# zero-savvy/vimz

Measured on AMD Instinct MI355X. Metric: nova_folding_steps_per_sec, higher is better.
Workload: dtype u32 limbs (256-bit Montgomery integers over BN254 Fr/Fq)

## Files before the change

vimz_amd/csrc/ec_mem.hpp:

```cpp
#pragma once
#include <hip/hip_runtime.h>
#include "ec.hpp"

namespace vz {

template <class F>
__device__ __forceinline__ void load_words20(const uint32_t* __restrict__ p, F& a, F& b) {
  const uint4* q = reinterpret_cast<const uint4*>(p);
  const uint4 w0 = q[0], w1 = q[1], w2 = q[2], w3 = q[3], w4 = q[4];
  a.v[0] = w0.x; a.v[1] = w0.y; a.v[2] = w0.z; a.v[3] = w0.w; a.v[4] = w1.x; a.v[5] = w1.y; a.v[6] = w1.z; a.v[7] = w1.w; a.v[8] = w2.x;
  b.v[0] = w2.z; b.v[1] = w2.w; b.v[2] = w3.x; b.v[3] = w3.y; b.v[4] = w3.z; b.v[5] = w3.w; b.v[6] = w4.x; b.v[7] = w4.y; b.v[8] = w4.z;
}
template <class F>
__device__ __forceinline__ void store_words20(uint32_t* __restrict__ p, const F& a, const F& b) {
  uint4* q = reinterpret_cast<uint4*>(p);
  q[0] = make_uint4(a.v[0], a.v[1], a.v[2], a.v[3]); q[1] = make_uint4(a.v[4], a.v[5], a.v[6], a.v[7]);
  q[2] = make_uint4(a.v[8], 0u, b.v[0], b.v[1]); q[3] = make_uint4(b.v[2], b.v[3], b.v[4], b.v[5]);
  q[4] = make_uint4(b.v[6], b.v[7], b.v[8], 0u);
}
struct RawAffine { uint4 w0, w1, w2, w3; };
__device__ __forceinline__ RawAffine load_affine_raw(const uint32_t* __restrict__ bases, size_t idx) {
  const uint4* q = reinterpret_cast<const uint4*>(bases + (size_t)AFFINE_WORDS * idx);
  RawAffine r; r.w0 = q[0]; r.w1 = q[1]; r.w2 = q[2]; r.w3 = q[3]; return r;
}
template <class F>
__device__ __forceinline__ Affine<F> affine_of_raw(const RawAffine& a) {
  const uint32_t x[8] = {a.w0.x, a.w0.y, a.w0.z, a.w0.w, a.w1.x, a.w1.y, a.w1.z, a.w1.w}, y[8] = {a.w2.x, a.w2.y, a.w2.z, a.w2.w, a.w3.x, a.w3.y, a.w3.z, a.w3.w};
  Affine<F> r; r.x = F::pack(x); r.y = F::pack(y); return r;
}
template <class F>
__device__ __forceinline__ Affine<F> load_affine_at(const uint32_t* __restrict__ p) { return affine_of_raw<F>(load_affine_raw(p, 0)); }
template <class F>
__device__ __forceinline__ Affine<F> load_affine(const uint32_t* __restrict__ bases, size_t idx) { return load_affine_at<F>(bases + (size_t)AFFINE_WORDS * idx); }
template <class F>
__device__ __forceinline__ void store_affine_at(uint32_t* __restrict__ p, const Affine<F>& a) {
  uint32_t x[8], y[8]; a.x.unpack(x); a.y.unpack(y);
  uint4* q = reinterpret_cast<uint4*>(p);
  q[0] = make_uint4(x[0], x[1], x[2], x[3]); q[1] = make_uint4(x[4], x[5], x[6], x[7]);
  q[2] = make_uint4(y[0], y[1], y[2], y[3]); q[3] = make_uint4(y[4], y[5], y[6], y[7]);
}
template <class F>
__device__ __forceinline__ void store_affine(uint32_t* __restrict__ bases, size_t idx, const Affine<F>& a) { store_affine_at<F>(bases + (size_t)AFFINE_WORDS * idx, a); }
constexpr int XYZZ_HALF_WORDS = 2 * COORD_WORDS;
template <class F>
__device__ __forceinline__ void store_xyzz(uint32_t* __restrict__ base, size_t idx, const XYZZ<F>& p) {
  uint32_t* d = base + (size_t)XYZZ_WORDS * idx;
  store_words20(d, p.X, p.Y); store_words20(d + XYZZ_HALF_WORDS, p.ZZ, p.ZZZ);
}
template <class F>
__device__ __forceinline__ XYZZ<F> load_xyzz(const uint32_t* __restrict__ base, size_t idx) {
  const uint32_t* d = base + (size_t)XYZZ_WORDS * idx;
  XYZZ<F> p; load_words20(d, p.X, p.Y); load_words20(d + XYZZ_HALF_WORDS, p.ZZ, p.ZZZ); return p;
}

template <class F> struct QuadRes { F c0, c1; XYZZ<F> full; uint32_t mode; };
template <int K, class F>
__device__ __forceinline__ F quad_bcast(const F& v) {
  F r;
#pragma unroll
  for (int i = 0; i < 9; i++) r.v[i] = (uint32_t)__builtin_amdgcn_update_dpp(0, (int)v.v[i], K * 0x55, 0xf, 0xf, true);
  return r;
}
template <class F>
__device__ __noinline__ void quad_add_rare(const XYZZ<F>* A, const XYZZ<F>* B, XYZZ<F>* out) { XYZZ<F> a = *A; add_full(a, *B); *out = a; }
template <class F>
__device__ __forceinline__ QuadRes<F> quad_add_compute(const XYZZ<F>* __restrict__ sh, uint32_t ia, uint32_t ib, bool active) {
  const int q = (int)(threadIdx.x & 3u);
  QuadRes<F> out; out.mode = 0;
  const XYZZ<F>& A = sh[ia]; const XYZZ<F>& B = sh[ib];
  const bool a_id = A.ZZ.is_zero(), b_id = B.ZZ.is_zero();
  auto sel = [](bool c, const F& x, const F& y) { F r; for (int i = 0; i < 9; i++) r.v[i] = c ? x.v[i] : y.v[i]; return r; };
  const F* px = q == 0 ? &A.X : q == 1 ? &B.X : q == 2 ? &A.Y : &B.Y;
  const F* py = q == 0 ? &B.ZZ : q == 1 ? &A.ZZ : q == 2 ? &B.ZZZ : &A.ZZZ;
  const F m1 = F::mul(*px, *py);
  F o1;
#pragma unroll
  for (int i = 0; i < 9; i++) o1.v[i] = (uint32_t)__builtin_amdgcn_update_dpp(0, (int)m1.v[i], 0xB1, 0xf, 0xf, true);
  const F lo = sel(q & 1, o1, m1), hi = sel(q & 1, m1, o1);
  const F PR = F::template sub<2>(hi, lo);
  const int pz = __builtin_amdgcn_update_dpp(0, (q == 0 && PR.is_zero_mod()) ? 1 : 0, 0x00, 0xf, 0xf, true);
  const F* pa = q == 1 ? &A.ZZ : &A.ZZZ; const F* pb = q == 1 ? &B.ZZ : &B.ZZZ;
  const F za = *pa, zb = *pb;
  const F m2 = F::mul(sel(q & 1, za, PR), sel(q & 1, zb, PR));
  const F PP = quad_bcast<0>(m2);
  const F Z12 = quad_bcast<1>(m2);
  const F m3 = F::mul(sel(q == 0, PR, sel(q == 1, lo, Z12)), PP);
  const F PPP = quad_bcast<0>(m3);
  const F Qv = quad_bcast<1>(m3);
  const F S1 = quad_bcast<2>(lo);
  const F X3 = F::template sub<4>(m2, F::add(PPP, F::dbl(Qv)));
  const F D = F::template sub<6>(Qv, X3);
  const F m4 = F::mul(sel(q == 0, S1, sel(q == 2, PR, m2)), sel(q == 2, D, PPP));
  const F Yb = quad_bcast<0>(m4);
  if (!active || b_id) return out;
  if (a_id) { out.mode = 1; out.c0 = q == 0 ? B.X : q == 1 ? B.Y : q == 2 ? B.ZZ : B.ZZZ; return out; }
  if (pz) {
    out.mode = 3;
    if (q == 0) { XYZZ<F> tmp; quad_add_rare<F>(&A, &B, &tmp); out.full = tmp; }
    return out;
  }
  out.mode = 2;
  if (q == 2) { out.c0 = X3; out.c1 = F::template sub<2>(m4, Yb); }
  if (q == 3) { out.c0 = m3; out.c1 = m4; }
  return out;
}
template <class F>
__device__ __forceinline__ void quad_add_store(XYZZ<F>* __restrict__ sh, uint32_t ia, const QuadRes<F>& r) {
  const int q = (int)(threadIdx.x & 3u);
  XYZZ<F>& A = sh[ia];
  if (r.mode == 1) { if (q == 0) A.X = r.c0; else if (q == 1) A.Y = r.c0; else if (q == 2) A.ZZ = r.c0; else A.ZZZ = r.c0; }
  else if (r.mode == 2) { if (q == 2) { A.X = r.c0; A.Y = r.c1; } else if (q == 3) { A.ZZ = r.c0; A.ZZZ = r.c1; } }
  else if (r.mode == 3 && q == 0) A = r.full;
}
template <class F, class Fd, class Fs>
__device__ __forceinline__ void quad_level(XYZZ<F>* __restrict__ sh, uint32_t count, Fd dst, Fs src) {
  const uint32_t e = threadIdx.x >> 2;
  const bool active = e < count;
  QuadRes<F> r; r.mode = 0;
  uint32_t ia = 0;
  const uint32_t wave0 = (uint32_t)__builtin_amdgcn_readfirstlane((int)(threadIdx.x & ~63u));
  if (wave0 < 4u * count) {
    ia = active ? dst(e) : 0u;
    const uint32_t ib = active ? src(e) : 0u;
    r = quad_add_compute<F>(sh, ia, ib, active);
  }
  __syncthreads();
  quad_add_store<F>(sh, ia, r);
  __syncthreads();
}

template <class F>
__device__ __forceinline__ void quad_tree256(XYZZ<F>* __restrict__ sh) {
  quad_level<F>(sh, 64, [](uint32_t e) { return e; }, [](uint32_t e) { return e + 128; });
  quad_level<F>(sh, 64, [](uint32_t e) { return e + 64; }, [](uint32_t e) { return e + 192; });
  for (uint32_t d = 64; d > 0; d >>= 1) quad_level<F>(sh, d, [](uint32_t e) { return e; }, [d](uint32_t e) { return e + d; });
}

}
```

vimz_amd/csrc/msm.hpp:

```cpp
#pragma once
#include <cstdlib>
#include <cstring>
#include <mutex>
#include "msm_api.hpp"
#include "ec_mem.hpp"

namespace vz {

struct MsmTuning { int sort_blocks = 0, combine_lane_bits = -1, small_lean = 0, witness_sub = 0, ones_dense = 1, reduce_planes = 0, accum_lds_kb = 0, dense_sub = 0, signed_scalars = 1; };
inline const MsmTuning& msm_tuning() {
  static const MsmTuning t = [] {
    MsmTuning r;
    if (const char* e = getenv("VIMZ_TUNE")) {
      if (const char* q = strstr(e, "sort_blocks=")) r.sort_blocks = atoi(q + 12);
      if (const char* q = strstr(e, "combine_lane_bits=")) r.combine_lane_bits = atoi(q + 18);
      if (const char* q = strstr(e, "small_lean=")) r.small_lean = atoi(q + 11);
      if (const char* q = strstr(e, "witness_sub=")) { const int v = atoi(q + 12); if (v >= 2 && v <= MSM_SUB) r.witness_sub = v; }
      if (const char* q = strstr(e, "dense_sub=")) { const int v = atoi(q + 10); if (v >= 2 && v <= MSM_SUB) r.dense_sub = v; }
      if (const char* q = strstr(e, "ones_dense=")) r.ones_dense = atoi(q + 11);
      if (const char* q = strstr(e, "reduce_planes=")) r.reduce_planes = atoi(q + 14);
      if (const char* q = strstr(e, "signed_scalars=")) r.signed_scalars = atoi(q + 15) != 0;
      if (const char* q = strstr(e, "accum_lds_kb=")) { const int v = atoi(q + 13); if (v >= 0 && v <= 160) r.accum_lds_kb = v; }
    }
    return r;
// ... 201 lines not shown
    for_each_digit(s, c, K, flip, [&](int w, uint32_t b, uint32_t neg) {
      const uint32_t pos = atomicAdd(&lds_pos[(uint32_t)w * nbw + b], 1u);
      sorted[pos] = ((uint32_t)i + (uint32_t)w * pt_stride) | (neg << 31);
    });
  }
}

template <class F>
__global__ void __launch_bounds__(256, 3) k_accum(const uint32_t* __restrict__ bases, const uint32_t* __restrict__ sorted,
                                               const uint32_t* __restrict__ bucket_off, const uint32_t* __restrict__ sub_off,
                                               uint32_t nb, const uint32_t* __restrict__ totals,
                                               uint32_t* __restrict__ partial, uint32_t sub) {
  const uint32_t total = totals[0];
  uint32_t s = blockIdx.x * blockDim.x + threadIdx.x;
  if (s >= total) return;
  uint32_t lo = 0, hi = nb;
  while (hi - lo > 1) {
    uint32_t mid = (lo + hi) >> 1;
    if (sub_off[mid] <= s) lo = mid; else hi = mid;
  }
  const uint32_t b = lo, k = s - sub_off[b];
  const uint32_t beg = bucket_off[b] + k * sub;
  const uint32_t end = min(bucket_off[b + 1], beg + sub);
  XYZZ<F> acc = XYZZ<F>::identity();
  uint32_t ent = beg < end ? sorted[beg] : 0u;
  RawAffine raw = load_affine_raw(bases, ent & 0x7fffffffu);
  for (uint32_t e = beg; e < end; e++) {
    const uint32_t ent_n = e + 1 < end ? sorted[e + 1] : ent;
    const RawAffine raw_n = load_affine_raw(bases, ent_n & 0x7fffffffu);
    Affine<F> q = affine_of_raw<F>(raw);
    if ((ent >> 31) && !aff_is_identity(q)) q.y = F::neg(q.y);
    add_mixed(acc, q);
    ent = ent_n; raw = raw_n;
  }
  store_xyzz(partial, s, acc);
}

constexpr uint32_t ONES_THREADS = 16384;
template <class S>
__device__ __forceinline__ bool scalar_is_one(const uint32_t* __restrict__ scalars, size_t i, int mont) {
  const uint4* p = reinterpret_cast<const uint4*>(scalars + 8 * i);
  const uint4 a = p[0], b = p[1];
  if (mont) return a.x == S::Params::R1.w[0] && a.y == S::Params::R1.w[1] && a.z == S::Params::R1.w[2] && a.w == S::Params::R1.w[3] &&
                   b.x == S::Params::R1.w[4] && b.y == S::Params::R1.w[5] && b.z == S::Params::R1.w[6] && b.w == S::Params::R1.w[7];
  return a.x == 1u && (a.y | a.z | a.w | b.x | b.y | b.z | b.w) == 0u;
}
template <class S, class F>
__global__ void __launch_bounds__(256) k_ones_partial(const uint32_t* __restrict__ scalars, const uint32_t* __restrict__ bases, size_t n, int mont,
                                                      uint32_t* __restrict__ out ) {
  const uint32_t t = blockIdx.x * blockDim.x + threadIdx.x;
  XYZZ<F> acc = XYZZ<F>::identity();
  for (size_t i = t; i < n; i += ONES_THREADS)
    if (scalar_is_one<S>(scalars, i, mont)) { Affine<F> q = load_affine<F>(bases, (uint32_t)i); add_mixed(acc, q); }
  store_xyzz(out, t, acc);
}
template <class S, class F>
__global__ void __launch_bounds__(256) k_ones_dense(const uint32_t* __restrict__ scalars, const uint32_t* __restrict__ bases, size_t n, int mont,
                                                    uint32_t* __restrict__ out ) {
  __shared__ uint32_t queue[4][128];
  const uint32_t t = blockIdx.x * blockDim.x + threadIdx.x, lane = threadIdx.x & 63u, wv = threadIdx.x >> 6;
  const size_t wave = t >> 6, nwaves = ONES_THREADS / 64;
  volatile uint32_t* q = queue[wv];
  XYZZ<F> acc = XYZZ<F>::identity();
  uint32_t cnt = 0;
  for (size_t base = wave * 64; base < n; base += nwaves * 64) {
    const size_t i = base + lane;
    const bool one = i < n && scalar_is_one<S>(scalars, i, mont);
    const uint64_t m = __ballot(one);
    if (one) q[cnt + (uint32_t)__popcll(m & ((1ull << lane) - 1ull))] = (uint32_t)i;
    cnt += (uint32_t)__popcll(m);
    __builtin_amdgcn_wave_barrier();
    if (cnt >= 64) {
      cnt -= 64;
      const uint32_t idx = q[cnt + lane];
      __builtin_amdgcn_wave_barrier();
      Affine<F> pt = load_affine<F>(bases, idx);
      add_mixed(acc, pt);
    }
  }
  if (lane < cnt) { Affine<F> pt = load_affine<F>(bases, q[lane]); add_mixed(acc, pt); }
  store_xyzz(out, t, acc);
}
template <class F>
__global__ void __launch_bounds__(256) k_tree256(const uint32_t* __restrict__ in, uint32_t m, uint32_t* __restrict__ out) {
  __shared__ XYZZ<F> sh[256];
  const uint32_t t = threadIdx.x, i = blockIdx.x * 256 + t;
  sh[t] = i < m ? load_xyzz<F>(in, i) : XYZZ<F>::identity();
  __syncthreads();
  quad_tree256<F>(sh);
  if (t == 0) store_xyzz(out, blockIdx.x, sh[0]);
}


constexpr uint32_t MSM_HEAVY_PARTS = 32, MSM_HEAVY_SPLIT = 1024;
constexpr uint32_t MSM_HEAVY_SPLIT_MIN = 2048;
constexpr uint32_t COMBINE_HEAVY_BLOCKS = 512, COMBINE_SPLIT_BLOCKS = 1024;

template <class F>
__global__ void __launch_bounds__(256) k_combine(uint32_t* __restrict__ partial, const uint32_t* __restrict__ sub_off, uint32_t nb, uint32_t nbn,
                                                 const uint32_t* __restrict__ heavy, uint32_t heavy_cap, uint32_t* scratch ,
                                                 uint32_t lane_bits , uint32_t heavy_min,
                                                 uint32_t* __restrict__ heavy_done ) {
  __shared__ XYZZ<F> sh[256];
  __shared__ uint32_t s_last;
  const uint32_t t = threadIdx.x;
  if (blockIdx.x < nbn) {
    const uint32_t L = 1u << lane_bits, lane = t & (L - 1u);
    const uint32_t b = blockIdx.x * (256u >> lane_bits) + (t >> lane_bits);
    uint32_t s0 = 0, m = 0;
    if (b < nb) { s0 = sub_off[b]; m = sub_off[b + 1] - s0; }
    if (m > heavy_min && heavy[0] <= heavy_cap) m = 0;
    if (!__syncthreads_or(m >= 2 ? 1 : 0)) return;
    XYZZ<F> acc = XYZZ<F>::identity();
    if (lane < m) acc = load_xyzz<F>(partial, s0 + lane);
    for (uint32_t k = lane + L; k < m; k += L) { XYZZ<F> q = load_xyzz<F>(partial, s0 + k); add_full(acc, q); }
    sh[t] = acc;
    __syncthreads();
    for (uint32_t d = L >> 1; d > 0; d >>= 1) {
      if (lane < d && lane + d < m) { XYZZ<F> a = sh[t]; add_full(a, sh[t + d]); sh[t] = a; }
      __syncthreads();
    }
    if (lane == 0 && m >= 2) store_xyzz(partial, s0, sh[t]);
    return;
  }
  const uint32_t count = heavy[0] <= heavy_cap ? heavy[0] : 0u;
  if (blockIdx.x < nbn + COMBINE_HEAVY_BLOCKS) {
    for (uint32_t h = blockIdx.x - nbn; h < count; h += COMBINE_HEAVY_BLOCKS) {
      const uint32_t b = heavy[1 + h];
      const uint32_t s0 = sub_off[b], m = sub_off[b + 1] - s0;
      if (h < MSM_HEAVY_SPLIT && m >= MSM_HEAVY_SPLIT_MIN) continue;
      XYZZ<F> acc = XYZZ<F>::identity();
      for (uint32_t k = t; k < m; k += 256) { XYZZ<F> q = load_xyzz<F>(partial, s0 + k); add_full(acc, q); }
      __syncthreads();
      sh[t] = acc;
      __syncthreads();
      quad_tree256<F>(sh);
      if (t == 0) store_xyzz(partial, s0, sh[0]);
    }
    return;
  }
  const uint32_t nsplit = min(count, MSM_HEAVY_SPLIT);
  for (uint32_t it = blockIdx.x - nbn - COMBINE_HEAVY_BLOCKS; it < nsplit * MSM_HEAVY_PARTS; it += COMBINE_SPLIT_BLOCKS) {
    const uint32_t b = heavy[1 + it / MSM_HEAVY_PARTS], part = it % MSM_HEAVY_PARTS;
    const uint32_t s0 = sub_off[b], m = sub_off[b + 1] - s0;
    if (m < MSM_HEAVY_SPLIT_MIN) continue;
    const uint32_t per = (m + MSM_HEAVY_PARTS - 1) / MSM_HEAVY_PARTS, lo = part * per, hi = min(m, lo + per);
    XYZZ<F> acc = XYZZ<F>::identity();
    for (uint32_t k = lo + t; k < hi; k += 256) { XYZZ<F> q = load_xyzz<F>(partial, s0 + k); add_full(acc, q); }
    __syncthreads();
    sh[t] = acc;
    __syncthreads();
    quad_tree256<F>(sh);
    if (t == 0) store_xyzz(scratch, it, sh[0]);
    const uint32_t hsl = it / MSM_HEAVY_PARTS;
    if (t == 0) { __threadfence(); s_last = atomicAdd(&heavy_done[hsl], 1u) == MSM_HEAVY_PARTS - 1 ? 1u : 0u; }
    __syncthreads();
    if (s_last) {
      __threadfence();
      if (t == 0) __hip_atomic_store(&heavy_done[hsl], 0u, __ATOMIC_RELAXED, __HIP_MEMORY_SCOPE_AGENT);
      sh[t] = t < MSM_HEAVY_PARTS ? load_xyzz<F>(scratch, (size_t)hsl * MSM_HEAVY_PARTS + t) : XYZZ<F>::identity();
      __syncthreads();
      for (uint32_t d = MSM_HEAVY_PARTS / 2; d > 0; d >>= 1) quad_level<F>(sh, d, [](uint32_t e) { return e; }, [d](uint32_t e) { return e + d; });
      if (t == 0) store_xyzz(partial, s0, sh[0]);
    }
    __syncthreads();
  }
}

template <class F>
__global__ void __launch_bounds__(256) k_reduce(const uint32_t* __restrict__ partial, const uint32_t* __restrict__ counts,
                                                const uint32_t* __restrict__ sub_off, uint32_t nbw,
                                                uint32_t* __restrict__ window_sums, uint32_t* __restrict__ plain_sums = nullptr) {
  __shared__ XYZZ<F> sh[256];
  const uint32_t w = blockIdx.x, t = threadIdx.x, T = blockDim.x;
  const uint32_t ch = nbw / T;
  const uint32_t lo = t * ch;
  XYZZ<F> run = XYZZ<F>::identity(), sum = XYZZ<F>::identity();
  for (uint32_t j = ch; j-- > 0;) {
    uint32_t g = w * nbw + lo + j;
    if (counts[g]) { XYZZ<F> B = load_xyzz<F>(partial, sub_off[g]); add_full(run, B); }
    add_full(sum, run);
  }
  sh[t] = run;
  __syncthreads();
  for (uint32_t d = 1; d < T; d <<= 1) {
    const bool act = t + d < T;
    XYZZ<F> o = XYZZ<F>::identity();
    if (act) o = sh[t + d];
    __syncthreads();
    if (act) { XYZZ<F> a = sh[t]; add_full(a, o); sh[t] = a; }
    __syncthreads();
  }
  if (t >= 1) {
    XYZZ<F> sfx = sh[t];
    for (uint32_t k = 1; k < ch; k <<= 1) sfx = dbl(sfx);
    add_full(sum, sfx);
  } else if (plain_sums) store_xyzz(plain_sums, w, sh[0]);
  __syncthreads();
  sh[t] = sum;
  __syncthreads();
  if (T == 256) quad_tree256<F>(sh);
  else for (uint32_t d = T >> 1; d > 0; d >>= 1) {
    if (t < d) { XYZZ<F> a = sh[t]; add_full(a, sh[t + d]); sh[t] = a; }
    __syncthreads();
  }
  if (t == 0) store_xyzz(window_sums, w, sh[0]);
}


template <class F>
__global__ void __launch_bounds__(256) k_reduce_planes(const uint32_t* __restrict__ partial, const uint32_t* __restrict__ counts, const uint32_t* __restrict__ sub_off,
                                                       uint32_t nbw, uint32_t P , uint32_t G , uint32_t lpt,
                                                       uint32_t* stage , uint32_t* __restrict__ ticket,
                                                       uint32_t* __restrict__ out ) {
  __shared__ XYZZ<F> sh[256];
  __shared__ uint32_t s_last;
  const uint32_t t = threadIdx.x, plane = blockIdx.x / G, q = blockIdx.x % G;
  XYZZ<F> acc = XYZZ<F>::identity();
  for (uint32_t i = 0; i < lpt; i++) {
    const uint32_t j = q * (256u * lpt) + i * 256u + t;
    uint32_t g;
    if (plane < P) g = ((j >> plane) << (plane + 1)) | (1u << plane) | (j & ((1u << plane) - 1u));
    else g = (plane - P) * (nbw >> 1) + j;
    if (counts[g]) { XYZZ<F> B = load_xyzz<F>(partial, sub_off[g]); add_full(acc, B); }
  }
  sh[t] = acc;
  __syncthreads();
  quad_tree256<F>(sh);
  if (t == 0) { store_xyzz(stage, blockIdx.x, sh[0]); __threadfence(); s_last = atomicAdd(ticket, 1u) == gridDim.x - 1 ? 1u : 0u; }
  __syncthreads();
  if (!s_last) return;
  __threadfence();
  if (t == 0) __hip_atomic_store(ticket, 0u, __ATOMIC_RELAXED, __HIP_MEMORY_SCOPE_AGENT);
  const uint32_t total = (P + 2) * G;
  sh[t] = t < total ? load_xyzz<F>(stage, t) : XYZZ<F>::identity();
  __syncthreads();
  for (uint32_t d = G >> 1; d > 0; d >>= 1) {
    const uint32_t pairs = (P + 2) * d;
    for (uint32_t base = 0; base < pairs; base += 64)
      quad_level<F>(sh, min(64u, pairs - base), [=](uint32_t e) { return ((base + e) / d) * G + (base + e) % d; }, [=](uint32_t e) { return ((base + e) / d) * G + (base + e) % d + d; });
  }
  if (t < P + 2) store_xyzz(out, t, sh[t * G]);
}

constexpr uint32_t SMALL_THREADS = 256;
constexpr uint32_t SMALL_NBW = 1u << (SMALL_C - 1), SMALL_SUB = 8 , SMALL_PER_THREAD = SMALL_CHUNK / SMALL_THREADS;
static_assert(SMALL_CHUNK / SMALL_SUB + SMALL_NBW <= SMALL_THREADS, "one thread per sub-bucket");
static_assert(SMALL_NBW == 64, "k_msm_small scans the buckets of a window with one wave");

template <int C>
struct DigitThreshold {
  uint32_t w[8];
  constexpr DigitThreshold() : w{} { for (int p = C - 1; p < 256; p += C) w[p >> 5] |= 1u << (p & 31); }
};
template <int C>
__device__ __forceinline__ int signed_digit(const uint32_t* s, int w) {
  constexpr DigitThreshold<C> T{};
  const int lo = C * w;
  uint32_t br = 0;
#pragma unroll
  for (int i = 0; i < 8; i++) {
    const int nb = lo - 32 * i;
    const uint32_t m = nb >= 32 ? 0xffffffffu : nb <= 0 ? 0u : (1u << nb) - 1u;
    const uint64_t d = (uint64_t)(T.w[i] & m) - (uint64_t)(s[i] & m) - br;
    br = (uint32_t)(d >> 63);
  }
  const uint32_t d = window_bits(s, lo, C) + br;
  return d > (1u << (C - 1)) ? (int)d - (1 << C) : (int)d;
}

template <class S, class F, int LEAN >
__global__ void __launch_bounds__(SMALL_THREADS) k_msm_small(const uint32_t* __restrict__ bases, const uint32_t* __restrict__ scalars, uint32_t n, int mont, int sgn,
                                                   uint32_t Q, uint32_t chunk, uint32_t* __restrict__ chunk_out ,
                                                   uint32_t* __restrict__ done ,
                                                   uint32_t* __restrict__ window_sums,
                                                   const uint32_t* __restrict__ tables , uint32_t tstride) {
  constexpr int lean = LEAN;
  __shared__ XYZZ<F> sh[SMALL_THREADS];
  __shared__ uint32_t cnt[SMALL_NBW], off[SMALL_NBW + 1], soff[SMALL_NBW + 1], cur[SMALL_NBW];
  __shared__ uint16_t list[SMALL_CHUNK];
  __shared__ uint8_t subb[SMALL_THREADS];
  __shared__ uint32_t s_maxm, s_ticket, wcnt[SMALL_THREADS / 64];
  VZ_SET_CRIT_PRIO();
  const uint32_t t = threadIdx.x, w = blockIdx.x, q = blockIdx.y;
  const uint32_t lo = q * chunk, hi = min(n, lo + chunk);
  const uint32_t* __restrict__ wbases = tables ? tables + (size_t)AFFINE_WORDS * ((size_t)w * tstride) : bases;
  if (t < SMALL_NBW) { cnt[t] = 0; cur[t] = 0; }
  __syncthreads();
  int dig[SMALL_PER_THREAD];
#pragma unroll
  for (int k = 0; k < (int)SMALL_PER_THREAD; k++) {
    dig[k] = 0;
    const uint32_t i = lo + t + SMALL_THREADS * k;
    if (i < hi) {
      uint32_t sc[8], flip;
      if (load_scalar<S>(scalars, i, mont, 0, sgn, sc, flip)) {
        dig[k] = signed_digit<SMALL_C>(sc, (int)w);
        if (flip) dig[k] = -dig[k];
        if (dig[k]) atomicAdd(&cnt[(dig[k] < 0 ? -dig[k] : dig[k]) - 1], 1u);
      }
    }
  }
  __syncthreads();
  if (t < 64) {
    const uint32_t c0 = cnt[t];
    uint32_t m4 = (c0 + 3) / 4, m5 = (c0 + 4) / 5, m6 = (c0 + 5) / 6, m7 = (c0 + 6) / 7;
    for (int o = 32; o > 0; o >>= 1) { m4 += __shfl_xor(m4, o); m5 += __shfl_xor(m5, o); m6 += __shfl_xor(m6, o); m7 += __shfl_xor(m7, o); }
    const uint32_t sub = m4 <= SMALL_THREADS ? 4u : m5 <= SMALL_THREADS ? 5u : m6 <= SMALL_THREADS ? 6u : m7 <= SMALL_THREADS ? 7u : 8u;
    const uint32_t m = (c0 + sub - 1) / sub;
    uint32_t ic = c0, im = m, mx = m;
    for (int o = 1; o < 64; o <<= 1) {
      const uint32_t uc = __shfl_up(ic, o), um = __shfl_up(im, o);
      if ((int)t >= o) { ic += uc; im += um; }
    }
    for (int o = 32; o > 0; o >>= 1) mx = max(mx, (uint32_t)__shfl_xor(mx, o));
    off[t] = ic - c0; soff[t] = im - m;
    if (t == 63) { off[SMALL_NBW] = ic; soff[SMALL_NBW] = im; s_maxm = mx; }
  }
  __syncthreads();
#pragma unroll
  for (int k = 0; k < (int)SMALL_PER_THREAD; k++) {
    if (dig[k]) {
      const uint32_t b = (uint32_t)(dig[k] < 0 ? -dig[k] : dig[k]) - 1;
      const uint32_t pos = atomicAdd(&cur[b], 1u);
      list[off[b] + pos] = (uint16_t)((t + SMALL_THREADS * k) | (dig[k] < 0 ? 0x8000u : 0u));
    }
  }
  if (t < SMALL_NBW) for (uint32_t sb = soff[t]; sb < soff[t + 1]; sb++) subb[sb] = (uint8_t)t;
  __syncthreads();
  const uint32_t nsubs = soff[SMALL_NBW];
  XYZZ<F> acc = XYZZ<F>::identity();
  uint32_t kk = 0, mb = 0;
  if (t < nsubs) {
    const uint32_t b = subb[t];
    kk = t - soff[b]; mb = soff[b + 1] - soff[b];
    const uint32_t cb = off[b + 1] - off[b];
    const uint32_t beg = off[b] + kk * cb / mb, end = off[b] + (kk + 1) * cb / mb;
    uint32_t ent = beg < end ? list[beg] : 0u;
    Affine<F> pt = load_affine<F>(wbases, lo + (ent & 0x7fffu));
    for (uint32_t e = beg; e < end; e++) {
      const uint32_t ent_n = e + 1 < end ? list[e + 1] : ent;
      const Affine<F> pt_n = load_affine<F>(wbases, lo + (ent_n & 0x7fffu));
      if ((ent & 0x8000u) && !aff_is_identity(pt)) pt.y = F::neg(pt.y);
      add_mixed(acc, pt);
      ent = ent_n; pt = pt_n;
    }
  }
  sh[t] = acc;
  __syncthreads();
  for (uint32_t d = 1; d < s_maxm; d <<= 1) {
    const bool act = t < nsubs && (kk & (2 * d - 1)) == 0 && kk + d < mb;
    const uint64_t bal = __ballot(act);
    if ((t & 63) == 0) wcnt[t >> 6] = (uint32_t)__popcll(bal);
    __syncthreads();
    uint32_t before = 0, total = 0;
    for (uint32_t wv = 0; wv < SMALL_THREADS / 64; wv++) { before += wv < (t >> 6) ? wcnt[wv] : 0u; total += wcnt[wv]; }
    if (act) list[before + (uint32_t)__popcll(bal & ((1ull << (t & 63)) - 1ull))] = (uint16_t)t;
    __syncthreads();
    if (lean && total >= 48) {
      const uint32_t wave0 = (uint32_t)__builtin_amdgcn_readfirstlane((int)(t & ~63u));
      XYZZ<F> a; uint32_t ia = 0; bool mine = false;
      if (wave0 < total) {
        mine = t < total;
        if (mine) { ia = list[t]; a = sh[ia]; add_full(a, sh[ia + d]); }
      }
      __syncthreads();
      if (mine) sh[ia] = a;
      __syncthreads();
    } else
    for (uint32_t base = 0; base < total; base += 64)
      quad_level<F>(sh, min(64u, total - base), [&](uint32_t e) { return (uint32_t)list[base + e]; }, [&](uint32_t e) { return (uint32_t)list[base + e] + d; });
  }
  XYZZ<F> bk = XYZZ<F>::identity();
  if (t < SMALL_NBW && cnt[t]) bk = sh[soff[t]];
  __syncthreads();
  if (Q > 1 && done) {
    if (t < SMALL_NBW) {
      store_xyzz(chunk_out, ((size_t)w * Q + q) * SMALL_NBW + t, bk);
      __threadfence();
      if (t == 0) s_ticket = atomicAdd(&done[w], 1u);
    }
    __syncthreads();
    if (s_ticket != Q - 1) return;
    __threadfence();

    const uint32_t b = t & (SMALL_NBW - 1), sl = t / SMALL_NBW;
    for (uint32_t loaded = 0; loaded < Q;) {
      const uint32_t slot0 = loaded ? 1u : 0u, k = min(Q - loaded, 4u - slot0), m = slot0 + k;
      if (sl >= slot0 && sl < m) {
        sh[t] = load_xyzz<F>(chunk_out, ((size_t)w * Q + loaded + sl - slot0) * SMALL_NBW + b);
      }
      __syncthreads();
      if (lean) {
        if ((sl == 0 && m >= 2) || (sl == 2 && m == 4)) { XYZZ<F> a = sh[t]; add_full(a, sh[t + SMALL_NBW]); sh[t] = a; }
        __syncthreads();
        if (sl == 0 && m >= 3) { XYZZ<F> a = sh[t]; add_full(a, sh[t + 2 * SMALL_NBW]); sh[t] = a; }
        __syncthreads();
      } else {
      if (m >= 2) quad_level<F>(sh, SMALL_NBW, [](uint32_t e) { return e; }, [](uint32_t e) { return e + SMALL_NBW; });
      if (m == 4) quad_level<F>(sh, SMALL_NBW, [](uint32_t e) { return e + 2 * SMALL_NBW; }, [](uint32_t e) { return e + 3 * SMALL_NBW; });
      if (m >= 3) quad_level<F>(sh, SMALL_NBW, [](uint32_t e) { return e; }, [](uint32_t e) { return e + 2 * SMALL_NBW; });
      }
      loaded += k;
    }
    if (t == 0) __hip_atomic_store(&done[w], 0u, __ATOMIC_RELAXED, __HIP_MEMORY_SCOPE_AGENT);
  } else {
    if (t < SMALL_NBW) sh[t] = bk;
    __syncthreads();
  }
  if (lean >= 2) {
    for (uint32_t d = 1; d < SMALL_NBW; d <<= 1) {
      XYZZ<F> a; const bool mine = t < SMALL_NBW - d;
      if (t < 64) { if (mine) { a = sh[t]; add_full(a, sh[t + d]); } }
      __syncthreads();
      if (mine) sh[t] = a;
      __syncthreads();
    }
  } else
  for (uint32_t d = 1; d < SMALL_NBW; d <<= 1)
    quad_level<F>(sh, SMALL_NBW - d, [](uint32_t e) { return e; }, [d](uint32_t e) { return e + d; });
  for (uint32_t d = SMALL_NBW / 2; d > 0; d >>= 1)
    quad_level<F>(sh, d, [](uint32_t e) { return e; }, [d](uint32_t e) { return e + d; });
  if (Q == 1 || done) { if (t == 0) store_xyzz(window_sums, w, sh[0]); return; }
  if (t == 0) store_xyzz(chunk_out, (size_t)w * Q + q, sh[0]);
}

template <class F>
__global__ void __launch_bounds__(64) k_msm_small_sum(const uint32_t* __restrict__ chunk_out, uint32_t Q, uint32_t* __restrict__ window_sums) {
  __shared__ XYZZ<F> sh[SMALL_MAXQ];
  const uint32_t t = threadIdx.x, w = blockIdx.x;
  if (t < SMALL_MAXQ) sh[t] = t < Q ? load_xyzz<F>(chunk_out, (size_t)w * Q + t) : XYZZ<F>::identity();
  __syncthreads();
  for (uint32_t d = SMALL_MAXQ / 2; d > 0; d >>= 1) {
    if (t < d) { XYZZ<F> a = sh[t]; add_full(a, sh[t + d]); sh[t] = a; }
    __syncthreads();
  }
  if (t == 0) store_xyzz(window_sums, w, sh[0]);
}

constexpr uint32_t FIXED_PER_THREAD = 4, FIXED_CHUNK = 256 * FIXED_PER_THREAD, FIXED_MAXQ = 64;
static_assert(MSM_SMALL_MAX <= (size_t)FIXED_CHUNK * FIXED_MAXQ, "a window's workgroup sums fit one tree");

template <class F>
__global__ void __launch_bounds__(256) k_build_multiples(const uint32_t* __restrict__ tables, size_t n, int K, uint32_t nm, uint32_t* __restrict__ mult) {
  const size_t g = blockIdx.x * (size_t)blockDim.x + threadIdx.x;
  if (g >= n * (size_t)K) return;
  const Affine<F> B = load_affine<F>(tables, (uint32_t)g);
  XYZZ<F> acc = from_affine(B);
  uint32_t* dst = mult + (size_t)AFFINE_WORDS * (g * nm);
  for (uint32_t m = 0; m < nm; m++) {
    const Affine<F> a = to_affine(acc);
    store_affine_at<F>(dst + (size_t)AFFINE_WORDS * m, a);
    add_mixed(acc, B);
  }
}
template <class C>
hipError_t build_multiples(hipStream_t stream, const uint32_t* d_tables, size_t n, int c, int K, uint32_t* d_mult) {
  typedef typename C::Coord F;
  if (!n) return hipSuccess;
  if (n * (size_t)K >= (1u << 31)) return hipErrorInvalidValue;
  hipLaunchKernelGGL(k_build_multiples<F>, dim3((unsigned)((n * (size_t)K + 255) / 256)), dim3(256), 0, stream, d_tables, n, K, 1u << (c - 1), d_mult);
  return hipGetLastError();
}

template <class S, class F>
__global__ void __launch_bounds__(256) k_msm_fixed(const uint32_t* __restrict__ mult, uint32_t tstride, const uint32_t* __restrict__ scalars, uint32_t n, int mont, int sgn,
                                                   uint32_t Q, uint32_t* __restrict__ partial , uint32_t* __restrict__ done ,
                                                   uint32_t* __restrict__ window_sums) {
  __shared__ XYZZ<F> sh[256];
  __shared__ uint32_t s_ticket;
  VZ_SET_CRIT_PRIO();
  const uint32_t t = threadIdx.x, q = blockIdx.x, w = blockIdx.y;
  constexpr uint32_t NM = SMALL_NBW;
  Affine<F> pt[FIXED_PER_THREAD];
  bool neg[FIXED_PER_THREAD], have[FIXED_PER_THREAD];
#pragma unroll
  for (int k = 0; k < (int)FIXED_PER_THREAD; k++) {
    const uint32_t i = q * FIXED_CHUNK + t + 256u * k;
    have[k] = false; neg[k] = false;
    if (i < n) {
      uint32_t sc[8], flip;
      if (load_scalar<S>(scalars, i, mont, 0, sgn, sc, flip)) {
        const int d = flip ? -signed_digit<SMALL_C>(sc, (int)w) : signed_digit<SMALL_C>(sc, (int)w);
        if (d) {
          have[k] = true; neg[k] = d < 0;
          const uint32_t m = (uint32_t)(d < 0 ? -d : d) - 1u;
          const uint32_t* src = mult + (size_t)AFFINE_WORDS * (((size_t)w * tstride + i) * NM + m);
          pt[k] = load_affine_at<F>(src);
        }
      }
    }
  }
  XYZZ<F> acc = XYZZ<F>::identity();
#pragma unroll
  for (int k = 0; k < (int)FIXED_PER_THREAD; k++) {
    if (have[k]) {
      if (neg[k] && !aff_is_identity(pt[k])) pt[k].y = F::neg(pt[k].y);
      add_mixed(acc, pt[k]);
    }
  }
  sh[t] = acc;
  __syncthreads();
  quad_level<F>(sh, 64, [](uint32_t e) { return e; }, [](uint32_t e) { return e + 128; });
  quad_level<F>(sh, 64, [](uint32_t e) { return e + 64; }, [](uint32_t e) { return e + 192; });
  for (uint32_t d = 64; d > 0; d >>= 1) quad_level<F>(sh, d, [](uint32_t e) { return e; }, [d](uint32_t e) { return e + d; });
  if (Q == 1) { if (t == 0) store_xyzz(window_sums, w, sh[0]); return; }
  if (t < 64) {
    if (t == 0) store_xyzz(partial, (size_t)w * Q + q, sh[0]);
    __threadfence();
    if (t == 0) s_ticket = atomicAdd(&done[w], 1u);
  }
  __syncthreads();
  if (s_ticket != Q - 1) return;
  __threadfence();
  if (t < FIXED_MAXQ) {
    XYZZ<F> v = XYZZ<F>::identity();
    if (t < Q) {
      v = load_xyzz<F>(partial, (size_t)w * Q + t);
    }
    sh[t] = v;
  }
  __syncthreads();
  uint32_t top = 1; while (top < Q) top <<= 1;
  for (uint32_t d = top >> 1; d > 0; d >>= 1) quad_level<F>(sh, d, [](uint32_t e) { return e; }, [d](uint32_t e) { return e + d; });
  if (t == 0) { store_xyzz(window_sums, w, sh[0]); __hip_atomic_store(&done[w], 0u, __ATOMIC_RELAXED, __HIP_MEMORY_SCOPE_AGENT); }
}



template <class F>
__device__ __forceinline__ XYZZ<F> small_mul(const XYZZ<F>& p, uint32_t k) {
  XYZZ<F> acc = XYZZ<F>::identity();
  if (!k) return acc;
  for (int bit = 31 - __clz(k); bit >= 0; bit--) { acc = dbl(acc); if ((k >> bit) & 1) add_full(acc, p); }
  return acc;
}
template <class F>
__global__ void __launch_bounds__(256) k_build_tables(const uint32_t* __restrict__ bases, size_t n, int c, int K, uint32_t* __restrict__ tables) {
  const size_t i = blockIdx.x * (size_t)blockDim.x + threadIdx.x;
  if (i >= n) return;
  Affine<F> p = load_affine<F>(bases, (uint32_t)i);
  store_affine<F>(tables, i, p);
  for (int j = 1; j < K; j++) {
    XYZZ<F> acc = from_affine(p);
    for (int k = 0; k < c; k++) acc = dbl(acc);
    p = to_affine(acc);
    store_affine<F>(tables, (size_t)j * n + i, p);
  }
}
template <class C>
hipError_t build_tables(hipStream_t stream, const uint32_t* d_bases, size_t n, int c, int K, uint32_t* d_tables) {
  typedef typename C::Coord F;
  if (!n) return hipSuccess;
  hipLaunchKernelGGL(k_build_tables<F>, dim3((unsigned)((n + 255) / 256)), dim3(256), 0, stream, d_bases, n, c, K, d_tables);
  return hipGetLastError();
}

template <class C>
hipError_t msm_launch(hipStream_t stream, MsmWorkspace& ws, const uint32_t* d_bases, const uint32_t* d_scalars, size_t n,
                      int scalars_mont, int c_override, void* pinned_dst, MsmPlan* plan_out, hipEvent_t* ev, int split_ones,
                      const BaseTables* tb) {
  typedef typename C::Coord F;
  typedef typename C::Scalar S;
  if (n == 0 || n >= (1u << 31)) return hipErrorInvalidValue;
  const int sgn = msm_tuning().signed_scalars;
  constexpr bool direct = true;
  static const bool no_small = getenv("VIMZ_DEBUG_NO_SMALL_MSM") != nullptr;
  const bool small_fmt = tb && tb->d && tb->c == SMALL_C;
  const bool small_tb = small_fmt && !no_small && c_override <= 0;
  bool tabled = tb && tb->d && !small_fmt && c_override <= 0;
  if (tabled && tb->own && tb->c != msm_plan(n, S::Params::BITS, 0).c) tabled = false;
  const bool own = tabled && tb->own;
  if (small_tb && (n > MSM_SMALL_MAX || tb->K != (S::Params::BITS + SMALL_C) / SMALL_C)) return hipErrorInvalidValue;
  if (!no_small && !tabled && c_override <= 0 && n <= MSM_SMALL_MAX) {
    MsmPlan ps; ps.c = SMALL_C; ps.K = (S::Params::BITS + SMALL_C) / SMALL_C; ps.nbw = SMALL_NBW; ps.nb = SMALL_NBW * (uint32_t)ps.K; ps.split_ones = 0; ps.tabled = small_tb ? 2 : 0;
    *plan_out = ps;
    VZ_HIP_CHECK(ws.reserve_small());
    const uint32_t Q = (uint32_t)((n + SMALL_CHUNK - 1) / SMALL_CHUNK), chunk = (uint32_t)((n + Q - 1) / Q);
    uint32_t* done = reinterpret_cast<uint32_t*>(ws.small_buf);
    uint32_t* chunk_out = done + 128;
    if (small_tb && tb->mult) {
      const uint32_t Qf = (uint32_t)((n + FIXED_CHUNK - 1) / FIXED_CHUNK);
      if (ev) for (int i = 0; i < 4; i++) VZ_HIP_CHECK(hipEventRecord(ev[i], stream));
      hipLaunchKernelGGL((k_msm_fixed<S, F>), dim3(Qf, ps.K), dim3(256), 0, stream, tb->mult + (size_t)AFFINE_WORDS * SMALL_NBW * tb->offset, (uint32_t)tb->n_total, d_scalars, (uint32_t)n,
                         scalars_mont, sgn, Qf, chunk_out, done, direct ? reinterpret_cast<uint32_t*>(pinned_dst) : reinterpret_cast<uint32_t*>(ws.window_sums));
      if (ev) for (int i = 4; i < 7; i++) VZ_HIP_CHECK(hipEventRecord(ev[i], stream));
      VZ_HIP_CHECK(hipGetLastError());
      if (!direct) VZ_HIP_CHECK(hipMemcpyAsync(pinned_dst, ws.window_sums, 4 * (size_t)XYZZ_WORDS * ps.K, hipMemcpyDeviceToHost, stream));
      return hipSuccess;
    }
    if (ev) for (int i = 0; i < 4; i++) VZ_HIP_CHECK(hipEventRecord(ev[i], stream));
    static const bool sum_kernel = getenv("VIMZ_DEBUG_SMALL_SUM_KERNEL") != nullptr;
#define VZ_SMALL(LEAN) hipLaunchKernelGGL((k_msm_small<S, F, LEAN>), dim3(ps.K, Q), dim3(SMALL_THREADS), 0, stream, d_bases, d_scalars, (uint32_t)n, scalars_mont, sgn, Q, chunk, chunk_out, \
                       sum_kernel ? (uint32_t*)nullptr : done, direct ? reinterpret_cast<uint32_t*>(pinned_dst) : reinterpret_cast<uint32_t*>(ws.window_sums), \
                       small_tb ? tb->d + (size_t)AFFINE_WORDS * tb->offset : (const uint32_t*)nullptr, small_tb ? (uint32_t)tb->n_total : 0u)
    switch (msm_tuning().small_lean) { case 0: VZ_SMALL(0); break; case 1: VZ_SMALL(1); break; default: VZ_SMALL(2); break; }
#undef VZ_SMALL
    if (Q > 1 && sum_kernel) hipLaunchKernelGGL(k_msm_small_sum<F>, dim3(ps.K), dim3(64), 0, stream, chunk_out, Q, direct ? reinterpret_cast<uint32_t*>(pinned_dst) : reinterpret_cast<uint32_t*>(ws.window_sums));
    if (ev) for (int i = 4; i < 7; i++) VZ_HIP_CHECK(hipEventRecord(ev[i], stream));
    VZ_HIP_CHECK(hipGetLastError());
    if (!direct) VZ_HIP_CHECK(hipMemcpyAsync(pinned_dst, ws.window_sums, 4 * (size_t)XYZZ_WORDS * ps.K, hipMemcpyDeviceToHost, stream));
    return hipSuccess;
  }
  MsmPlan pl = msm_plan(n, S::Params::BITS, tabled ? tb->c : c_override);
  if (tabled) {
    if (tb->K != pl.K || pl.nbw < 256 || (size_t)tb->K * tb->n_total >= (1u << 31)) return hipErrorInvalidValue;
    if (!own && 2 * (pl.nbw / std::min<uint32_t>(pl.nbw, MSM_VWIN)) + 1 > (uint32_t)MSM_MAX_WINDOWS) return hipErrorInvalidValue;
// ... 188 lines not shown
```

Measured before the change: 1360.

## Defer rare doubling case in quad tree adds to shared queue, shrink code

The quad-cooperative XYZZ add used to handle the equal-points case inline with a noinline full add, and each result struct carried a whole XYZZ point. Such cases are now pushed onto a 64-entry shared-memory queue and handled after the barrier by a few threads with add_full. This shrinks the per-thread result state and the register pressure. Tree levels become rolled loops (unroll 1) to cut code size, and several kernels get occupancy hints in launch_bounds. The cost is an extra read of the queue counter per level, plus possible slowdowns if the occupancy hints cause register spills.

```diff
diff --git a/vimz_amd/csrc/ec_mem.hpp b/vimz_amd/csrc/ec_mem.hpp
--- a/vimz_amd/csrc/ec_mem.hpp
+++ b/vimz_amd/csrc/ec_mem.hpp
@@ -53,7 +53,7 @@
   XYZZ<F> p; load_words20(d, p.X, p.Y); load_words20(d + XYZZ_HALF_WORDS, p.ZZ, p.ZZZ); return p;
 }
 
-template <class F> struct QuadRes { F c0, c1; XYZZ<F> full; uint32_t mode; };
+template <class F> struct QuadRes { F c0, c1; uint32_t mode; };
 template <int K, class F>
 __device__ __forceinline__ F quad_bcast(const F& v) {
   F r;
@@ -61,10 +61,13 @@
   for (int i = 0; i < 9; i++) r.v[i] = (uint32_t)__builtin_amdgcn_update_dpp(0, (int)v.v[i], K * 0x55, 0xf, 0xf, true);
   return r;
 }
+struct QuadQueue { uint32_t total; uint32_t ent[64]; };
+struct QuadCtx {
+  QuadQueue& q; uint32_t seen;
+  __device__ __forceinline__ explicit QuadCtx(QuadQueue& queue) : q(queue), seen(0) { if (threadIdx.x == 0) q.total = 0; }
+};
 template <class F>
-__device__ __noinline__ void quad_add_rare(const XYZZ<F>* A, const XYZZ<F>* B, XYZZ<F>* out) { XYZZ<F> a = *A; add_full(a, *B); *out = a; }
-template <class F>
-__device__ __forceinline__ QuadRes<F> quad_add_compute(const XYZZ<F>* __restrict__ sh, uint32_t ia, uint32_t ib, bool active) {
+__device__ __forceinline__ QuadRes<F> quad_add_compute(const XYZZ<F>* __restrict__ sh, QuadQueue& qq, uint32_t ia, uint32_t ib, bool active) {
   const int q = (int)(threadIdx.x & 3u);
   QuadRes<F> out; out.mode = 0;
   const XYZZ<F>& A = sh[ia]; const XYZZ<F>& B = sh[ib];
@@ -95,8 +98,7 @@
   if (!active || b_id) return out;
   if (a_id) { out.mode = 1; out.c0 = q == 0 ? B.X : q == 1 ? B.Y : q == 2 ? B.ZZ : B.ZZZ; return out; }
   if (pz) {
-    out.mode = 3;
-    if (q == 0) { XYZZ<F> tmp; quad_add_rare<F>(&A, &B, &tmp); out.full = tmp; }
+    if (q == 0) { const uint32_t pos = atomicAdd(&qq.total, 1u); qq.ent[pos & 63u] = ia | (ib << 16); }
     return out;
   }
   out.mode = 2;
@@ -110,10 +112,9 @@
   XYZZ<F>& A = sh[ia];
   if (r.mode == 1) { if (q == 0) A.X = r.c0; else if (q == 1) A.Y = r.c0; else if (q == 2) A.ZZ = r.c0; else A.ZZZ = r.c0; }
   else if (r.mode == 2) { if (q == 2) { A.X = r.c0; A.Y = r.c1; } else if (q == 3) { A.ZZ = r.c0; A.ZZZ = r.c1; } }
-  else if (r.mode == 3 && q == 0) A = r.full;
 }
 template <class F, class Fd, class Fs>
-__device__ __forceinline__ void quad_level(XYZZ<F>* __restrict__ sh, uint32_t count, Fd dst, Fs src) {
+__device__ __forceinline__ void quad_level(XYZZ<F>* __restrict__ sh, QuadCtx& qc, uint32_t count, Fd dst, Fs src) {
   const uint32_t e = threadIdx.x >> 2;
   const bool active = e < count;
   QuadRes<F> r; r.mode = 0;
@@ -122,18 +123,34 @@
   if (wave0 < 4u * count) {
     ia = active ? dst(e) : 0u;
     const uint32_t ib = active ? src(e) : 0u;
-    r = quad_add_compute<F>(sh, ia, ib, active);
+    r = quad_add_compute<F>(sh, qc.q, ia, ib, active);
   }
   __syncthreads();
-  quad_add_store<F>(sh, ia, r);
+  const uint32_t total = (uint32_t)__builtin_amdgcn_readfirstlane((int)*(volatile uint32_t*)&qc.q.total);
+  const uint32_t pending = total - qc.seen;
+  if (__builtin_expect(pending != 0u, 0)) {
+    XYZZ<F> a; uint32_t fa = 0;
+    const bool mine = threadIdx.x < pending;
+    if (mine) {
+      const uint32_t ent = qc.q.ent[(qc.seen + threadIdx.x) & 63u];
+      fa = ent & 0xffffu;
+      a = sh[fa]; add_full(a, sh[ent >> 16]);
+    }
+    __syncthreads();
+    quad_add_store<F>(sh, ia, r);
+    if (mine) sh[fa] = a;
+    qc.seen = total;
+  } else quad_add_store<F>(sh, ia, r);
   __syncthreads();
 }
 
 template <class F>
-__device__ __forceinline__ void quad_tree256(XYZZ<F>* __restrict__ sh) {
-  quad_level<F>(sh, 64, [](uint32_t e) { return e; }, [](uint32_t e) { return e + 128; });
-  quad_level<F>(sh, 64, [](uint32_t e) { return e + 64; }, [](uint32_t e) { return e + 192; });
-  for (uint32_t d = 64; d > 0; d >>= 1) quad_level<F>(sh, d, [](uint32_t e) { return e; }, [d](uint32_t e) { return e + d; });
+__device__ __forceinline__ void quad_tree256(XYZZ<F>* __restrict__ sh, QuadCtx& qc, uint32_t first = 0) {
+#pragma unroll 1
+  for (uint32_t lv = first; lv < 9; lv++) {
+    const uint32_t d = lv < 2 ? 128u : 256u >> lv, o = lv == 1 ? 64u : 0u;
+    quad_level<F>(sh, qc, min(d, 64u), [o](uint32_t e) { return e + o; }, [o, d](uint32_t e) { return e + o + d; });
+  }
 }
 
 }
diff --git a/vimz_amd/csrc/msm.hpp b/vimz_amd/csrc/msm.hpp
--- a/vimz_amd/csrc/msm.hpp
+++ b/vimz_amd/csrc/msm.hpp
@@ -307,12 +307,14 @@
   store_xyzz(out, t, acc);
 }
 template <class F>
-__global__ void __launch_bounds__(256) k_tree256(const uint32_t* __restrict__ in, uint32_t m, uint32_t* __restrict__ out) {
+__global__ void __launch_bounds__(256, 4) k_tree256(const uint32_t* __restrict__ in, uint32_t m, uint32_t* __restrict__ out) {
   __shared__ XYZZ<F> sh[256];
+  __shared__ QuadQueue qq;
+  QuadCtx qc(qq);
   const uint32_t t = threadIdx.x, i = blockIdx.x * 256 + t;
   sh[t] = i < m ? load_xyzz<F>(in, i) : XYZZ<F>::identity();
   __syncthreads();
-  quad_tree256<F>(sh);
+  quad_tree256<F>(sh, qc);
   if (t == 0) store_xyzz(out, blockIdx.x, sh[0]);
 }
 
@@ -322,12 +324,14 @@
 constexpr uint32_t COMBINE_HEAVY_BLOCKS = 512, COMBINE_SPLIT_BLOCKS = 1024;
 
 template <class F>
-__global__ void __launch_bounds__(256) k_combine(uint32_t* __restrict__ partial, const uint32_t* __restrict__ sub_off, uint32_t nb, uint32_t nbn,
+__global__ void __launch_bounds__(256, 3) k_combine(uint32_t* __restrict__ partial, const uint32_t* __restrict__ sub_off, uint32_t nb, uint32_t nbn,
                                                  const uint32_t* __restrict__ heavy, uint32_t heavy_cap, uint32_t* scratch ,
                                                  uint32_t lane_bits , uint32_t heavy_min,
                                                  uint32_t* __restrict__ heavy_done ) {
   __shared__ XYZZ<F> sh[256];
   __shared__ uint32_t s_last;
+  __shared__ QuadQueue qq;
+  QuadCtx qc(qq);
   const uint32_t t = threadIdx.x;
   if (blockIdx.x < nbn) {
     const uint32_t L = 1u << lane_bits, lane = t & (L - 1u);
@@ -359,7 +363,7 @@
       __syncthreads();
       sh[t] = acc;
       __syncthreads();
-      quad_tree256<F>(sh);
+      quad_tree256<F>(sh, qc);
       if (t == 0) store_xyzz(partial, s0, sh[0]);
     }
     return;
@@ -375,7 +379,7 @@
     __syncthreads();
     sh[t] = acc;
     __syncthreads();
-    quad_tree256<F>(sh);
+    quad_tree256<F>(sh, qc);
     if (t == 0) store_xyzz(scratch, it, sh[0]);
     const uint32_t hsl = it / MSM_HEAVY_PARTS;
     if (t == 0) { __threadfence(); s_last = atomicAdd(&heavy_done[hsl], 1u) == MSM_HEAVY_PARTS - 1 ? 1u : 0u; }
@@ -385,7 +389,8 @@
       if (t == 0) __hip_atomic_store(&heavy_done[hsl], 0u, __ATOMIC_RELAXED, __HIP_MEMORY_SCOPE_AGENT);
       sh[t] = t < MSM_HEAVY_PARTS ? load_xyzz<F>(scratch, (size_t)hsl * MSM_HEAVY_PARTS + t) : XYZZ<F>::identity();
       __syncthreads();
-      for (uint32_t d = MSM_HEAVY_PARTS / 2; d > 0; d >>= 1) quad_level<F>(sh, d, [](uint32_t e) { return e; }, [d](uint32_t e) { return e + d; });
+      static_assert(MSM_HEAVY_PARTS == 32, "the last five levels of the tree");
+      quad_tree256<F>(sh, qc, 4);
       if (t == 0) store_xyzz(partial, s0, sh[0]);
     }
     __syncthreads();
@@ -393,10 +398,12 @@
 }
 
 template <class F>
-__global__ void __launch_bounds__(256) k_reduce(const uint32_t* __restrict__ partial, const uint32_t* __restrict__ counts,
+__global__ void __launch_bounds__(256, 3) k_reduce(const uint32_t* __restrict__ partial, const uint32_t* __restrict__ counts,
                                                 const uint32_t* __restrict__ sub_off, uint32_t nbw,
                                                 uint32_t* __restrict__ window_sums, uint32_t* __restrict__ plain_sums = nullptr) {
   __shared__ XYZZ<F> sh[256];
+  __shared__ QuadQueue qq;
+  QuadCtx qc(qq);
   const uint32_t w = blockIdx.x, t = threadIdx.x, T = blockDim.x;
   const uint32_t ch = nbw / T;
   const uint32_t lo = t * ch;
@@ -424,7 +431,7 @@
   __syncthreads();
   sh[t] = sum;
   __syncthreads();
-  if (T == 256) quad_tree256<F>(sh);
+  if (T == 256) quad_tree256<F>(sh, qc);
   else for (uint32_t d = T >> 1; d > 0; d >>= 1) {
     if (t < d) { XYZZ<F> a = sh[t]; add_full(a, sh[t + d]); sh[t] = a; }
     __syncthreads();
@@ -434,12 +441,14 @@
 
 
 template <class F>
-__global__ void __launch_bounds__(256) k_reduce_planes(const uint32_t* __restrict__ partial, const uint32_t* __restrict__ counts, const uint32_t* __restrict__ sub_off,
+__global__ void __launch_bounds__(256, 3) k_reduce_planes(const uint32_t* __restrict__ partial, const uint32_t* __restrict__ counts, const uint32_t* __restrict__ sub_off,
                                                        uint32_t nbw, uint32_t P , uint32_t G , uint32_t lpt,
                                                        uint32_t* stage , uint32_t* __restrict__ ticket,
                                                        uint32_t* __restrict__ out ) {
   __shared__ XYZZ<F> sh[256];
   __shared__ uint32_t s_last;
+  __shared__ QuadQueue qq;
+  QuadCtx qc(qq);
   const uint32_t t = threadIdx.x, plane = blockIdx.x / G, q = blockIdx.x % G;
   XYZZ<F> acc = XYZZ<F>::identity();
   for (uint32_t i = 0; i < lpt; i++) {
@@ -451,7 +460,7 @@
   }
   sh[t] = acc;
   __syncthreads();
-  quad_tree256<F>(sh);
+  quad_tree256<F>(sh, qc);
   if (t == 0) { store_xyzz(stage, blockIdx.x, sh[0]); __threadfence(); s_last = atomicAdd(ticket, 1u) == gridDim.x - 1 ? 1u : 0u; }
   __syncthreads();
   if (!s_last) return;
@@ -460,10 +469,12 @@
   const uint32_t total = (P + 2) * G;
   sh[t] = t < total ? load_xyzz<F>(stage, t) : XYZZ<F>::identity();
   __syncthreads();
+#pragma unroll 1
   for (uint32_t d = G >> 1; d > 0; d >>= 1) {
     const uint32_t pairs = (P + 2) * d;
+#pragma unroll 1
     for (uint32_t base = 0; base < pairs; base += 64)
-      quad_level<F>(sh, min(64u, pairs - base), [=](uint32_t e) { return ((base + e) / d) * G + (base + e) % d; }, [=](uint32_t e) { return ((base + e) / d) * G + (base + e) % d + d; });
+      quad_level<F>(sh, qc, min(64u, pairs - base), [=](uint32_t e) { return ((base + e) / d) * G + (base + e) % d; }, [=](uint32_t e) { return ((base + e) / d) * G + (base + e) % d + d; });
   }
   if (t < P + 2) store_xyzz(out, t, sh[t * G]);
 }
@@ -495,7 +506,7 @@
 }
 
 template <class S, class F, int LEAN >
-__global__ void __launch_bounds__(SMALL_THREADS) k_msm_small(const uint32_t* __restrict__ bases, const uint32_t* __restrict__ scalars, uint32_t n, int mont, int sgn,
+__global__ void __launch_bounds__(SMALL_THREADS, 3) k_msm_small(const uint32_t* __restrict__ bases, const uint32_t* __restrict__ scalars, uint32_t n, int mont, int sgn,
                                                    uint32_t Q, uint32_t chunk, uint32_t* __restrict__ chunk_out ,
                                                    uint32_t* __restrict__ done ,
                                                    uint32_t* __restrict__ window_sums,
@@ -506,6 +517,8 @@
   __shared__ uint16_t list[SMALL_CHUNK];
   __shared__ uint8_t subb[SMALL_THREADS];
   __shared__ uint32_t s_maxm, s_ticket, wcnt[SMALL_THREADS / 64];
+  __shared__ QuadQueue qq;
+  QuadCtx qc(qq);
   VZ_SET_CRIT_PRIO();
   const uint32_t t = threadIdx.x, w = blockIdx.x, q = blockIdx.y;
   const uint32_t lo = q * chunk, hi = min(n, lo + chunk);
@@ -573,6 +586,7 @@
   }
   sh[t] = acc;
   __syncthreads();
+#pragma unroll 1
   for (uint32_t d = 1; d < s_maxm; d <<= 1) {
     const bool act = t < nsubs && (kk & (2 * d - 1)) == 0 && kk + d < mb;
     const uint64_t bal = __ballot(act);
@@ -593,8 +607,9 @@
       if (mine) sh[ia] = a;
       __syncthreads();
     } else
+#pragma unroll 1
     for (uint32_t base = 0; base < total; base += 64)
-      quad_level<F>(sh, min(64u, total - base), [&](uint32_t e) { return (uint32_t)list[base + e]; }, [&](uint32_t e) { return (uint32_t)list[base + e] + d; });
+      quad_level<F>(sh, qc, min(64u, total - base), [&](uint32_t e) { return (uint32_t)list[base + e]; }, [&](uint32_t e) { return (uint32_t)list[base + e] + d; });
   }
   XYZZ<F> bk = XYZZ<F>::identity();
   if (t < SMALL_NBW && cnt[t]) bk = sh[soff[t]];
@@ -622,9 +637,12 @@
         if (sl == 0 && m >= 3) { XYZZ<F> a = sh[t]; add_full(a, sh[t + 2 * SMALL_NBW]); sh[t] = a; }
         __syncthreads();
       } else {
-      if (m >= 2) quad_level<F>(sh, SMALL_NBW, [](uint32_t e) { return e; }, [](uint32_t e) { return e + SMALL_NBW; });
-      if (m == 4) quad_level<F>(sh, SMALL_NBW, [](uint32_t e) { return e + 2 * SMALL_NBW; }, [](uint32_t e) { return e + 3 * SMALL_NBW; });
-      if (m >= 3) quad_level<F>(sh, SMALL_NBW, [](uint32_t e) { return e; }, [](uint32_t e) { return e + 2 * SMALL_NBW; });
+#pragma unroll 1
+      for (uint32_t st = 0; st < 3; st++) {
+        const bool go = st == 0 ? m >= 2 : st == 1 ? m == 4 : m >= 3;
+        const uint32_t od = st == 1 ? 2 * SMALL_NBW : 0u, os = st == 0 ? SMALL_NBW : st == 1 ? 3 * SMALL_NBW : 2 * SMALL_NBW;
+        if (go) quad_level<F>(sh, qc, SMALL_NBW, [od](uint32_t e) { return e + od; }, [os](uint32_t e) { return e + os; });
+      }
       }
       loaded += k;
     }
@@ -641,11 +659,12 @@
       if (mine) sh[t] = a;
       __syncthreads();
     }
-  } else
-  for (uint32_t d = 1; d < SMALL_NBW; d <<= 1)
-    quad_level<F>(sh, SMALL_NBW - d, [](uint32_t e) { return e; }, [d](uint32_t e) { return e + d; });
-  for (uint32_t d = SMALL_NBW / 2; d > 0; d >>= 1)
-    quad_level<F>(sh, d, [](uint32_t e) { return e; }, [d](uint32_t e) { return e + d; });
+  }
+#pragma unroll 1
+  for (uint32_t lv = lean >= 2 ? 6u : 0u; lv < 12; lv++) {
+    const uint32_t d = lv < 6 ? 1u << lv : 32u >> (lv - 6), count = lv < 6 ? SMALL_NBW - d : d;
+    quad_level<F>(sh, qc, count, [](uint32_t e) { return e; }, [d](uint32_t e) { return e + d; });
+  }
   if (Q == 1 || done) { if (t == 0) store_xyzz(window_sums, w, sh[0]); return; }
   if (t == 0) store_xyzz(chunk_out, (size_t)w * Q + q, sh[0]);
 }
@@ -694,6 +713,8 @@
                                                    uint32_t* __restrict__ window_sums) {
   __shared__ XYZZ<F> sh[256];
   __shared__ uint32_t s_ticket;
+  __shared__ QuadQueue qq;
+  QuadCtx qc(qq);
   VZ_SET_CRIT_PRIO();
   const uint32_t t = threadIdx.x, q = blockIdx.x, w = blockIdx.y;
   constexpr uint32_t NM = SMALL_NBW;
@@ -726,9 +747,7 @@
   }
   sh[t] = acc;
   __syncthreads();
-  quad_level<F>(sh, 64, [](uint32_t e) { return e; }, [](uint32_t e) { return e + 128; });
-  quad_level<F>(sh, 64, [](uint32_t e) { return e + 64; }, [](uint32_t e) { return e + 192; });
-  for (uint32_t d = 64; d > 0; d >>= 1) quad_level<F>(sh, d, [](uint32_t e) { return e; }, [d](uint32_t e) { return e + d; });
+  quad_tree256<F>(sh, qc);
   if (Q == 1) { if (t == 0) store_xyzz(window_sums, w, sh[0]); return; }
   if (t < 64) {
     if (t == 0) store_xyzz(partial, (size_t)w * Q + q, sh[0]);
@@ -747,7 +766,8 @@
   }
   __syncthreads();
   uint32_t top = 1; while (top < Q) top <<= 1;
-  for (uint32_t d = top >> 1; d > 0; d >>= 1) quad_level<F>(sh, d, [](uint32_t e) { return e; }, [d](uint32_t e) { return e + d; });
+#pragma unroll 1
+  for (uint32_t d = top >> 1; d > 0; d >>= 1) quad_level<F>(sh, qc, d, [](uint32_t e) { return e; }, [d](uint32_t e) { return e + d; });
   if (t == 0) { store_xyzz(window_sums, w, sh[0]); __hip_atomic_store(&done[w], 0u, __ATOMIC_RELAXED, __HIP_MEMORY_SCOPE_AGENT); }
 }
 
```

New measurement: 1329. 0.977x the previous value.
